# saandeepa93/distributed_compute_pytorch

Measured on AMD Instinct MI355X. Metric: samples/sec (whole node) ResNet-50 DDP at 1/2/4/8 MI355X; scaling efficiency, higher is better.
Workload: dtype bf16; 1 GPU; model=resnet50, global_batch=1024, per_gpu_batch=1024, grad_accum=1, parallelism=dp1, impl=ours, fused_kernels=True, optimizer=SGD, comm_dtype=fp32, hip_graph=False, grad_to_none=True, backend=rccl, mfma_1x1_gemm=True, image_size=224, channels_last=True, res_prologue=False

## Files before the change

csrc/fused.cpp:

```cpp
#include "fused.h"

#include <cstring>

#include <c10/hip/HIPGuard.h>
#include <c10/hip/HIPStream.h>

#include <map>
#include <tuple>
#include <mutex>

#include "common.h"
#include "kernels/bn_kernels.h"
#include "kernels/gemm_kernels.h"
#include "kernels/attn_kernels.h"
#include "kernels/kernels.h"
#include "kernels/ln_kernels.h"
#include "kernels/dropout_kernels.h"
#include "kernels/pool_kernels.h"
#include "kernels/metrics_kernels.h"
#include "kernels/gelu_kernels.h"

namespace dcp {
namespace fused {

// ... 1096 lines not shown
  at::Tensor o = at::empty(q.sizes(), q.options().memory_format(at::MemoryFormat::Contiguous));
  at::Tensor lse = at::empty({q.size(0) * heads, q.size(1)}, q.options().dtype(at::kFloat));
  const bool store = p.p_drop > 0.f && keep_bits;
  at::Tensor mask = at::empty({store ? kern::attn_mask_words(p.B, p.H, p.T) : 0}, q.options().dtype(at::kInt));
  if (store) p.mask = reinterpret_cast<uint32_t*>(mask.data_ptr<int32_t>());
  kern::attn_fwd(p, attn_view(q, "q"), attn_view(k, "k"), attn_view(v, "v"), attn_out(o, "o"), lse.data_ptr<float>(),
                 stream_of(q));
  return {o, lse, mask};
}

void flash_attn_bwd(const at::Tensor& dout, const at::Tensor& q, const at::Tensor& k, const at::Tensor& v,
                    const at::Tensor& o, const at::Tensor& lse, const at::Tensor& mask, int64_t heads, bool causal,
                    double p_drop, int64_t seed, at::Tensor& dq, at::Tensor& dk, at::Tensor& dv,
                    const c10::optional<at::Tensor>& key_mask) {
  for (const at::Tensor* t : std::initializer_list<const at::Tensor*>{&k, &v, &o, &dout, &dq, &dk, &dv})
    same_shape(q, *t, "flash_attn_bwd");
  c10::hip::HIPGuard guard(q.device().index());
  kern::AttnParams p = attn_params(q, heads, causal, p_drop, seed);
  p.kmask = attn_kmask(key_mask, q, p, "flash_attn_bwd");
  DK_CHECK(lse.scalar_type() == at::kFloat && lse.is_contiguous() && lse.numel() == q.size(0) * heads * q.size(1),
            "flash_attn_bwd: lse");
  if (p.p_drop > 0.f) {
    DK_CHECK(mask.is_cuda() && mask.scalar_type() == at::kInt && mask.is_contiguous() &&
                 mask.numel() == kern::attn_mask_words(p.B, p.H, p.T),
             "flash_attn_bwd: dropout keep bits of the forward required");
    p.mask = reinterpret_cast<uint32_t*>(const_cast<int32_t*>(mask.data_ptr<int32_t>()));
  }
  at::Tensor delta = at::empty_like(lse);
  kern::attn_bwd(p, attn_view(q, "q"), attn_view(k, "k"), attn_view(v, "v"), attn_view(o, "o"),
                 attn_view(dout, "dout"), lse.data_ptr<float>(), delta.data_ptr<float>(), attn_out(dq, "dq"),
                 attn_out(dk, "dk"), attn_out(dv, "dv"), stream_of(q));
}

namespace {
float* fptr(const c10::optional<at::Tensor>& t) {
  return (t.has_value() && t->defined()) ? t->data_ptr<float>() : nullptr;
}
}

std::vector<at::Tensor> bn_resbn_act_fwd(const at::Tensor& x, const at::Tensor& weight, const at::Tensor& bias,
                                         const c10::optional<at::Tensor>& running_mean,
                                         const c10::optional<at::Tensor>& running_var,
                                         const c10::optional<at::Tensor>& nbt, const at::Tensor& stats,
                                         const at::Tensor& x2, const at::Tensor& weight2, const at::Tensor& bias2,
                                         const c10::optional<at::Tensor>& running_mean2,
                                         const c10::optional<at::Tensor>& running_var2,
                                         const c10::optional<at::Tensor>& nbt2, const at::Tensor& stats2,
                                         double momentum, double eps, double momentum2, double eps2) {
  check_nhwc(x, "bn_resbn_act_fwd");
  check_nhwc(x2, "bn_resbn_act_fwd(x2)");
  c10::hip::HIPGuard guard(x.device().index());
  const int64_t C = x.size(1);
  const int64_t M = x.numel() / C;
  DK_CHECK(x2.sizes() == x.sizes() && x2.scalar_type() == x.scalar_type(), "bn_resbn_act_fwd: x2 mismatch");
  for (const at::Tensor* t : {&stats, &stats2})
    DK_CHECK(t->scalar_type() == at::kFloat && t->numel() == 2 * C && t->is_contiguous(),
              "bn_resbn_act_fwd: stats must be fp32 [2*C]");
  for (const at::Tensor* t : {&weight, &bias, &weight2, &bias2})
    DK_CHECK(t->scalar_type() == at::kFloat && t->numel() == C && t->is_contiguous(),
              "bn_resbn_act_fwd: affine parameters must be fp32 [C]");
  auto fopt = x.options().dtype(at::kFloat);
  at::Tensor y = at::empty_like(x, cl_fmt(x));
  at::Tensor mean = at::empty({C}, fopt), invstd = at::empty({C}, fopt);
  at::Tensor mean2 = at::empty({C}, fopt), invstd2 = at::empty({C}, fopt);
  at::Tensor bits = at::empty({M * C / 8}, x.options().dtype(at::kByte));
  kern::ResBnArgs rb;
  rb.acc = stats2.data_ptr<float>();
  rb.gamma = weight2.data_ptr<float>();
  rb.beta = bias2.data_ptr<float>();
  rb.mean_out = mean2.data_ptr<float>();
  rb.invstd_out = invstd2.data_ptr<float>();
  rb.running_mean = fptr(running_mean2);
  rb.running_var = fptr(running_var2);
  rb.momentum = static_cast<float>(momentum2);
  rb.eps = static_cast<float>(eps2);
  rb.nbt = nbt2.has_value() && nbt2->defined() ? nbt2->data_ptr<int64_t>() : nullptr;
  kern::bn_forward_train_resbn(bn_dtype(x), x.data_ptr(), x2.data_ptr(), y.data_ptr(), M, static_cast<int>(C),
                               weight.data_ptr<float>(), bias.data_ptr<float>(), fptr(running_mean),
                               fptr(running_var), static_cast<float>(momentum), static_cast<float>(eps),
                               mean.data_ptr<float>(), invstd.data_ptr<float>(), stats.data_ptr<float>(),
                               nbt.has_value() && nbt->defined() ? nbt->data_ptr<int64_t>() : nullptr,
                               bits.data_ptr<uint8_t>(), rb, stream_of(x));
  return {y, mean, invstd, bits, mean2, invstd2};
}

std::vector<at::Tensor> bn_resbn_act_bwd(const at::Tensor& gy, const c10::optional<at::Tensor>& gy2_opt,
                                         const at::Tensor& x, const at::Tensor& weight, const at::Tensor& mean,
                                         const at::Tensor& invstd, const at::Tensor& bits, const at::Tensor& x2,
                                         const at::Tensor& weight2, const at::Tensor& mean2,
                                         const at::Tensor& invstd2) {
  check_nhwc(x, "bn_resbn_act_bwd");
  c10::hip::HIPGuard guard(x.device().index());
  at::Tensor g = gy.contiguous(cl_fmt(x));
  if (g.scalar_type() != x.scalar_type()) g = g.to(x.scalar_type());
  at::Tensor g2;
  if (gy2_opt.has_value() && gy2_opt->defined()) {
    g2 = gy2_opt->contiguous(cl_fmt(x));
    if (g2.scalar_type() != x.scalar_type()) g2 = g2.to(x.scalar_type());
  }
  const int64_t C = x.size(1);
  const int64_t M = x.numel() / C;
  DK_CHECK(bits.numel() == M * C / 8, "bn_resbn_act_bwd: relu bits mismatch");
  auto fopt = x.options().dtype(at::kFloat);
  auto s = stream_of(x);
  at::Tensor gout = at::empty_like(x, cl_fmt(x));
  at::Tensor dx = at::empty_like(x, cl_fmt(x)), dx2 = at::empty_like(x2, cl_fmt(x2));
  at::Tensor dw = at::empty({C}, fopt), db = at::empty({C}, fopt), dw2 = at::empty({C}, fopt),
             db2 = at::empty({C}, fopt);
  at::Tensor acc = zeroed_floats(2 * C, x, s), acc2 = zeroed_floats(2 * C, x, s);
  kern::bn_backward_resbn(bn_dtype(x), g.data_ptr(), g2.defined() ? g2.data_ptr() : nullptr, x.data_ptr(), M,
                          static_cast<int>(C), weight.data_ptr<float>(), mean.data_ptr<float>(),
                          invstd.data_ptr<float>(), bits.data_ptr<uint8_t>(), gout.data_ptr(), dx.data_ptr(),
                          dw.data_ptr<float>(), db.data_ptr<float>(), acc.data_ptr<float>(), x2.data_ptr(),
                          mean2.data_ptr<float>(), acc2.data_ptr<float>(), s);
  kern::bn_backward_apply_plain(bn_dtype(x), gout.data_ptr(), x2.data_ptr(), M, static_cast<int>(C),
                                weight2.data_ptr<float>(), mean2.data_ptr<float>(), invstd2.data_ptr<float>(),
                                acc2.data_ptr<float>(), dx2.data_ptr(), dw2.data_ptr<float>(),
                                db2.data_ptr<float>(), s);
  return {dx, dw, db, dx2, dw2, db2};
}

std::vector<at::Tensor> bn_act_bwd(const at::Tensor& gy, const c10::optional<at::Tensor>& gy2_opt,
                                   const at::Tensor& x, const c10::optional<at::Tensor>& weight,
                                   const c10::optional<at::Tensor>& bias, const at::Tensor& mean,
                                   const at::Tensor& invstd, const at::Tensor& y, bool act, bool has_res,
                                   bool training, const c10::optional<at::Tensor>& relu_bits) {
  check_nhwc(x, "bn_act_bwd");
  c10::hip::HIPGuard guard(x.device().index());
  at::Tensor g = gy.contiguous(cl_fmt(x));
  if (g.scalar_type() != x.scalar_type()) g = g.to(x.scalar_type());
  at::Tensor g2;
  if (gy2_opt.has_value() && gy2_opt->defined()) {
    g2 = gy2_opt->contiguous(cl_fmt(x));
    if (g2.scalar_type() != x.scalar_type()) g2 = g2.to(x.scalar_type());
    if (!has_res) {
      g = g + g2;
      g2 = at::Tensor();
    }
  }
  const int64_t C = x.size(1);
  const int64_t M = x.numel() / C;
  auto fopt = x.options().dtype(at::kFloat);
  at::Tensor dx = at::empty_like(x, cl_fmt(x));
  at::Tensor gres = has_res ? at::empty_like(x, cl_fmt(x)) : at::Tensor();
  const bool has_w = weight.has_value() && weight->defined();
  at::Tensor w = has_w ? weight->to(at::kFloat).contiguous() : at::Tensor();
  const bool has_bias = bias.has_value() && bias->defined();
  at::Tensor bf = has_bias ? bias->to(at::kFloat).contiguous() : at::Tensor();
  at::Tensor dw = at::empty({C}, fopt);
  at::Tensor db = at::empty({C}, fopt);
  at::Tensor acc = zeroed_floats(2 * C, x, stream_of(x));
  kern::bn_backward(bn_dtype(x), g.data_ptr(), g2.defined() ? g2.data_ptr() : nullptr, y.data_ptr(), x.data_ptr(),
                    M, static_cast<int>(C),
                    has_w ? w.data_ptr<float>() : nullptr, bf.defined() ? bf.data_ptr<float>() : nullptr,
                    mean.data_ptr<float>(), invstd.data_ptr<float>(), act,
                    has_res, has_res ? gres.data_ptr() : nullptr, dx.data_ptr(), dw.data_ptr<float>(),
                    db.data_ptr<float>(), acc.data_ptr<float>(), training,
                    relu_bits.has_value() && relu_bits->defined() && relu_bits->numel() == M * C / 8
                        ? relu_bits->data_ptr<uint8_t>()
                        : nullptr,
                    stream_of(x));
  at::Tensor dweight = has_w ? dw.to(weight->scalar_type()) : at::Tensor();
  const bool has_b = bias.has_value() && bias->defined();
  at::Tensor dbias = has_b ? db.to(bias->scalar_type()) : at::Tensor();
  return {dx, dweight, dbias, gres};
}
// ... 391 lines not shown
  m.def("bn_supported", [](int64_t C) { return kern::bn_supported(static_cast<int>(C)); });
  m.def("layer_norm_supported", &layer_norm_supported);
  m.def("linear_dgrad_gelu", &linear_dgrad_gelu, pybind11::arg("gy"), pybind11::arg("w2t"), pybind11::arg("h"),
        pybind11::arg("tanh_approx"), pybind11::arg("accumulate_into") = pybind11::none(),
        pybind11::arg("pp") = false);
  m.def("layer_norm_fwd", &layer_norm_fwd, pybind11::arg("x"), pybind11::arg("weight"), pybind11::arg("bias"),
        pybind11::arg("eps"), pybind11::arg("out_dtype") = pybind11::none(), pybind11::arg("branch") = pybind11::none(),
        pybind11::arg("p") = 0.0, pybind11::arg("seed") = 0, pybind11::arg("offset_dev") = pybind11::none());
  m.def("layer_norm_bwd", &layer_norm_bwd, pybind11::arg("dy"), pybind11::arg("x"), pybind11::arg("weight"),
        pybind11::arg("bias"), pybind11::arg("mean"), pybind11::arg("rstd"),
        pybind11::arg("accumulate_into") = pybind11::none(), pybind11::arg("grad_residual") = pybind11::none(),
        pybind11::arg("dy2") = pybind11::none(), pybind11::arg("drop_p") = 0.0, pybind11::arg("drop_seed") = 0,
        pybind11::arg("drop_offset_dev") = pybind11::none(), pybind11::arg("branch_grad") = false);
  m.def("cross_entropy_fwd", &cross_entropy_fwd, pybind11::arg("logits"), pybind11::arg("target"),
        pybind11::arg("ignore_index"), pybind11::arg("label_smoothing"), pybind11::arg("n_valid") = -1);
  m.def("log_softmax_fwd", &log_softmax_fwd, pybind11::arg("x"), pybind11::arg("out_dtype") = pybind11::none());
  m.def("log_softmax_bwd", &log_softmax_bwd);
  m.def("cross_entropy_bwd", &cross_entropy_bwd, pybind11::arg("logits"), pybind11::arg("target"),
        pybind11::arg("lse"), pybind11::arg("dloss"), pybind11::arg("ignore_index"), pybind11::arg("label_smoothing"),
        pybind11::arg("n_valid") = -1, pybind11::arg("inplace") = false);
  m.def("bn_act_fwd", &bn_act_fwd, "fused NHWC BatchNorm(+residual)(+ReLU) forward", pybind11::arg("x"),
        pybind11::arg("weight"), pybind11::arg("bias"), pybind11::arg("running_mean"), pybind11::arg("running_var"),
        pybind11::arg("residual"), pybind11::arg("training"), pybind11::arg("momentum"), pybind11::arg("eps"),
        pybind11::arg("act"), pybind11::arg("num_batches_tracked") = pybind11::none(),
        pybind11::arg("stats") = pybind11::none());
  m.def("bn_stats_coef", &bn_stats_coef, "training BN statistics + folded scale/shift (no apply)",
        pybind11::arg("x"), pybind11::arg("weight"), pybind11::arg("bias"), pybind11::arg("running_mean"),
        pybind11::arg("running_var"), pybind11::arg("momentum"), pybind11::arg("eps"),
        pybind11::arg("num_batches_tracked") = pybind11::none(), pybind11::arg("sums") = pybind11::none());
  m.def("conv1x1_supported", &conv1x1_supported);
  m.def("conv1x1_fwd", &conv1x1_fwd, "NHWC 1x1 conv as an MFMA GEMM (+BN-apply prologue, +BN-stats epilogue)",
        pybind11::arg("x"), pybind11::arg("w"), pybind11::arg("scale") = pybind11::none(),
        pybind11::arg("shift") = pybind11::none(), pybind11::arg("relu") = false, pybind11::arg("stats") = false);
  m.def("conv1x1_dgrad", &conv1x1_dgrad, pybind11::arg("gy"), pybind11::arg("wt"));
  m.def("conv1x1_fwd_res", &conv1x1_fwd_res, "block boundary: conv1x1(relu(x*scale+shift+res), w) with y and its "
        "ReLU mask stored by the GEMM's prologue", py::arg("x"), py::arg("w"), py::arg("scale"), py::arg("shift"),
        py::arg("res"), py::arg("stats") = true);
  m.def("lm_head_xent_fwd", &lm_head_xent_fwd,
        "LM head GEMM with the cross-entropy's softmax partials in its epilogue -> (logits, loss, lse)",
        py::arg("x"), py::arg("w"), py::arg("target"), py::arg("ignore_index"), py::arg("V"));
  m.def("gemm_pp", &gemm_pp, "x·wᵀ (+bias) (+gelu) on the 8-wave ping-pong 256x256 MFMA GEMM", py::arg("x"),
        py::arg("w"), py::arg("bias") = py::none(), py::arg("gelu") = 0);
  m.def("linear_fwd", &linear_fwd, "Linear forward on the MFMA GEMM: bias (+ GELU tanh/erf) in the epilogue",
        pybind11::arg("x"), pybind11::arg("w"), pybind11::arg("b"), pybind11::arg("gelu") = 0);
  m.def("attn_ok", &attn_ok);
  m.def("embedding_small_bwd", &embedding_small_bwd, "gw += per-index row sums (embedding tables of <= 8 rows)",
        pybind11::arg("idx"), pybind11::arg("g"), pybind11::arg("gw"));
  m.def("colsum", &colsum, "fp32 column sums of a bf16 [.., N] tensor (bias gradient)", pybind11::arg("x"),
        pybind11::arg("accumulate_into") = pybind11::none());
  m.def("colsum_multi", &colsum_multi, "colsum over 1-4 bf16 row segments in one launch", pybind11::arg("xs"),
        pybind11::arg("accumulate_into") = pybind11::none());
  m.def("gelu_fwd", &gelu_fwd, "bf16 GELU forward (erf or tanh form)", pybind11::arg("h"),
        pybind11::arg("tanh_approx"));
  m.def("gelu_bwd", &gelu_bwd, "bf16 GELU backward (+ fused bias-gradient column sums)", pybind11::arg("gy"),
        pybind11::arg("h"), pybind11::arg("tanh_approx"), pybind11::arg("bias_grad"),
        pybind11::arg("accumulate_into") = pybind11::none());
  m.def("flash_attn_fwd", &flash_attn_fwd, "MFMA flash attention forward (head dim 64)", pybind11::arg("q"),
        pybind11::arg("k"), pybind11::arg("v"), pybind11::arg("heads"), pybind11::arg("causal"),
        pybind11::arg("p_drop"), pybind11::arg("seed"), pybind11::arg("keep_bits") = true,
        pybind11::arg("key_mask") = pybind11::none());
  m.def("flash_attn_bwd", &flash_attn_bwd, "MFMA flash attention backward into dq/dk/dv", pybind11::arg("dout"),
        pybind11::arg("q"), pybind11::arg("k"), pybind11::arg("v"), pybind11::arg("o"), pybind11::arg("lse"),
        pybind11::arg("keep"), pybind11::arg("heads"), pybind11::arg("causal"), pybind11::arg("p_drop"),
        pybind11::arg("seed"), pybind11::arg("dq"), pybind11::arg("dk"), pybind11::arg("dv"),
        pybind11::arg("key_mask") = pybind11::none());
  m.def("attn_pack_key_mask", &attn_pack_key_mask,
        "bool [B, T] key-padding mask -> packed int64 [B, 1 + T/64] for flash_attn_fwd / flash_attn_bwd",
        pybind11::arg("mask"));
  m.def("conv_fwd", &conv_fwd, "kxk NHWC conv forward (implicit-GEMM MFMA) [+ output BN sums]", pybind11::arg("x"),
        pybind11::arg("wt"), pybind11::arg("kh"), pybind11::arg("kw"), pybind11::arg("stride"), pybind11::arg("pad"),
        pybind11::arg("stats") = false);
  m.def("conv1x1_dgrad_bnred", &conv1x1_dgrad_bnred, "1x1 data gradient + BN/ReLU backward reduction epilogue");
  m.def("conv_dgrad_bnred", &conv_dgrad_bnred, "stride-1 kxk data gradient + BN/ReLU backward reduction epilogue");
  m.def("conv1x1_dgrad_resred", &conv1x1_dgrad_resred,
        "1x1 data gradient + residual BN(+RBN)/ReLU backward reduction epilogue -> (g, acc, acc2)",
        pybind11::arg("gy"), pybind11::arg("wt"), pybind11::arg("x"), pybind11::arg("gy2"), pybind11::arg("mean"),
        pybind11::arg("bits"), pybind11::arg("x2") = pybind11::none(), pybind11::arg("mean2") = pybind11::none());
  m.def("bn_bwd_apply_g", &bn_bwd_apply_g, "BN training backward apply from a masked gradient + its reduction");
  m.def("conv3_bwd_fused", &conv3_bwd_fused,
        "bottleneck conv3 backward with BN3's backward apply as its prologue -> (dy2, acc2, dz3)");
  m.def("conv3_bwd_mode", [](int64_t M, int64_t w) { return kern::conv3_bwd_mode(M, static_cast<int>(w)); },
        "0: conv3's backward of this shape stays unfused; 1: conv3_bwd_fused");
  m.def("bn_dparams", &bn_dparams, "(dweight, dbias) of a training BN from its backward reduction");
  m.def("bn_bwd_apply2_g", &bn_bwd_apply2_g,
        "both BNs of relu(bn(x) + bn2(x2)) backward from the shared masked gradient in one pass");
  m.def("bn_act_bwd_apply", &bn_act_bwd_apply, "BN/ReLU training backward apply from a precomputed reduction");
  m.def("bn_resbn_act_fwd", &bn_resbn_act_fwd, "training relu(bn(x) + bn2(x2)), both BNs fused (downsample block)");
  m.def("bn_resbn_act_bwd", &bn_resbn_act_bwd, "backward of bn_resbn_act_fwd");
  m.def("conv1x1_s2_dgrad", &conv1x1_s2_dgrad, "stride-2 1x1 conv data gradient (GEMM + scattering epilogue)");
  m.def("conv_dgrad_s2_multi", &conv_dgrad_s2_multi,
        "3x3 stride-2 pad-1 conv data gradient: four parity classes in one implicit-GEMM launch");
  m.def("conv_dgrad_s2", &conv_dgrad_s2, "stride-2 kxk conv data gradient as four parity-class implicit GEMMs");
  m.def("conv_wgrad", &conv_wgrad, "kxk NHWC conv weight gradient (implicit-GEMM MFMA, fp32 out)",
        pybind11::arg("gy"), pybind11::arg("x"), pybind11::arg("kh"), pybind11::arg("kw"), pybind11::arg("stride"),
        pybind11::arg("pad"));
  m.def("weight_bf16_t", &weight_bf16_t, "fp32 weight -> (bf16 [R,C], bf16 transposed [C,R]) in one launch");
  m.def("conv_weight_bf16", &conv_weight_bf16, "kxk weight -> (bf16 fwd [Co][kh][kw][Ci], bf16 flipped [Ci][kh][kw][Co])");
  m.def("weight_prep_plan", &weight_prep_plan,
        "conv / Linear weights -> (device table, tiles, bf16 fwd views, bf16 dgrad views), one view pair per group "
        "(a group of Linear weights is packed along its rows)",
        py::arg("weights"), py::arg("groups") = std::vector<int64_t>{}, py::arg("pad_rows") = std::vector<int64_t>{});
  m.def("weight_prep_run", &weight_prep_run, py::arg("table"), py::arg("tiles"));
  m.def("conv1x1_wgrad", &conv1x1_wgrad, pybind11::arg("gy"), pybind11::arg("x"),
        pybind11::arg("scale") = pybind11::none(), pybind11::arg("shift") = pybind11::none(),
        pybind11::arg("relu") = false, pybind11::arg("accumulate_into") = pybind11::none(),
        pybind11::arg("out_rows") = -1, pybind11::arg("slots") = 0);
  m.def("conv1x1_wgrad_multi", &conv1x1_wgrad_multi,
        "dW = sum over 1-4 (gy, x) row segments (gradient-accumulation micro-steps) in one wgrad launch",
        pybind11::arg("gys"), pybind11::arg("xs"), pybind11::arg("accumulate_into") = pybind11::none(),
        pybind11::arg("out_rows") = -1);
  m.def("bn_act_bwd", &bn_act_bwd, "fused NHWC BatchNorm(+residual)(+ReLU) backward", pybind11::arg("gy"),
        pybind11::arg("gy2"), pybind11::arg("x"), pybind11::arg("weight"), pybind11::arg("bias"),
        pybind11::arg("mean"), pybind11::arg("invstd"), pybind11::arg("y"), pybind11::arg("act"),
        pybind11::arg("has_res"), pybind11::arg("training"), pybind11::arg("relu_bits") = pybind11::none());
}

}
}
```

csrc/kernels/gemm.hip:

```cpp
#include <hip/hip_runtime.h>

#include <cstdlib>
#include <string>

#include "gelu_math.h"
#include "gemm_kernels.h"
#include "kernels.h"
#include "stem_kernels.h"

namespace dcp {
namespace kern {
namespace {

typedef __bf16 bf16x8 __attribute__((ext_vector_type(8)));
typedef short s16x4 __attribute__((ext_vector_type(4)));
typedef short s16x8 __attribute__((ext_vector_type(8)));
typedef float f32x4 __attribute__((ext_vector_type(4)));
typedef __attribute__((address_space(3))) s16x4 lds_s16x4;

constexpr int kT = 256;
int g_wg_slots = 512;
int g_wg_cap = 0;
constexpr int kBK = 32;
constexpr int kNS = 4;
// ... 1518 lines not shown
        const int row = wi * 32 + i * 16 + (lane >> 4) * 4 + r;
        const int col = (j >> 1) * C + wj * 32 + (j & 1) * 16 + (lane & 15);
        out[static_cast<int64_t>(row) * COLS + col] = acc[i][j][r];
      }
}

struct WgradPlan {
  int bm, bn, tiles, S;
  int64_t chunk;
};

inline int wgrad_order() { return 1; }

inline bool wgrad_mtap(int N2, int taps) { return taps > 1 && N2 == 64; }

WgradPlan wgrad_plan(int64_t M, int N1, int N2, int taps = 1) {
  WgradPlan p;
  p.bm = N1 % 128 == 0 ? 128 : 64;
  p.bn = N2 % 128 == 0 ? 128 : 64;
  p.tiles = (N1 / p.bm) * (N2 / p.bn);
  constexpr int kStep = 64;
  const int64_t ksteps = (M + kStep - 1) / kStep;
  const int64_t slots = (g_wg_cap == 0 && taps > 1 && M <= 65536) ? 2 * g_wg_slots : g_wg_slots;
  int64_t S = slots / (p.tiles * taps);
  const int64_t capx = g_wg_cap > 0 ? g_wg_cap : (M <= 65536 ? 4 : 1);
  const int64_t cap = capx * (M * (N1 + static_cast<int64_t>(taps) * N2) * 2 / 2) /
                      (static_cast<int64_t>(N1) * taps * N2 * 4);
  if (S > cap) S = cap;
  if (S > ksteps) S = ksteps;
  if (S < 1) S = 1;
  p.chunk = ((ksteps + S - 1) / S) * kStep;
  p.S = static_cast<int>((M + p.chunk - 1) / p.chunk);
  return p;
}

}

bool gemm_nt_supported(int64_t M, int64_t N, int64_t K) {
  return M >= 1 && N > 0 && K > 0 && N % 64 == 0 && K % 64 == 0 && K <= 4096;
}

namespace {
inline int nt_bk() { return 64; }

inline int nt_bm(int64_t M, int tn, int BN, bool pro, int K, bool gather) {
  if (BN == 64) return !gather && K >= 256 ? 256 : 128;
  return pro && (M / 256) * tn >= 256 ? 256 : 128;
}

}

namespace {
int g_nt_big = 2;
int g_lin_big = 1;
int g_big_pipe = 0;
int g_nt_a = 0;
int g_stem_wide = 1;
int g_slab32 = 1;
int g_nt_deep = 0;
int g_pro_pipe = 0;
int g_reserve_cus = [] {
  const char* v = getenv("DCP_RESERVE_CUS");
  const int r = v ? atoi(v) : 0;
  return r < 0 ? 0 : (r > 192 ? 192 : r);
}();
inline int grid_cus() { return 256 - g_reserve_cus; }
}
void gemm_tune(const char* key, int value) {
  const std::string k(key);
  if (k == "nt_big") g_nt_big = value;
  if (k == "lin_big") g_lin_big = value;
  if (k == "big_pipe") g_big_pipe = value;
  if (k == "nt_a") g_nt_a = value < 0 ? 0 : (value > 3 ? 3 : value);
  if (k == "stem_wide") g_stem_wide = value;
  if (k == "slab32") g_slab32 = value;
  if (k == "nt_deep") g_nt_deep = value;
  if (k == "pro_pipe") g_pro_pipe = value;
  if (k == "wg_slots") g_wg_slots = value < 64 ? 64 : value;
  if (k == "wg_cap") g_wg_cap = value < 0 ? 0 : value;
  if (k == "reserve_cus") g_reserve_cus = value < 0 ? 0 : (value > 192 ? 192 : value);
  if (k.rfind("pp_", 0) == 0) gemm_pp_tune(key, value);
  if (k.rfind("bn_", 0) == 0) bn_tune(key, value);
  if (k.rfind("c3bwd", 0) == 0) conv3_bwd_tune(key, value);
  wgrad_pp_tune(key, value);
}
int gemm_tune_get(const char* key) {
  const std::string k(key);
  if (k == "nt_big") return g_nt_big;
  if (k == "lin_big") return g_lin_big;
  if (k == "big_pipe") return g_big_pipe;
  if (k == "nt_a") return g_nt_a;
  if (k == "stem_wide") return g_stem_wide;
  if (k == "slab32") return g_slab32;
  if (k == "nt_deep") return g_nt_deep;
  if (k == "pro_pipe") return g_pro_pipe;
  if (k == "wg_slots") return g_wg_slots;
  if (k == "wg_cap") return g_wg_cap;
  if (k == "reserve_cus") return g_reserve_cus;
  if (k.rfind("pp_", 0) == 0) return gemm_pp_tune_get(key);
  if (k.rfind("bn_", 0) == 0) return bn_tune_get(key);
  if (k.rfind("c3bwd", 0) == 0) return conv3_bwd_tune_get(key);
  return wgrad_pp_tune_get(key);
}

namespace {
template <bool GATHER, int BK, int BM>
void gemm_nt_launch_bm(const void* A, const void* B, void* C, int64_t M, int N, int K, const float* scale,
                       const float* shift, bool relu, float* stats, const ConvGeo& geo, const BnRedArgs* red,
                       hipStream_t s, bool scatter2, bool parity) {
  const int BN = N % 128 == 0 ? 128 : 64;
  const int tiles_m = static_cast<int>((M + BM - 1) / BM);
  const int tn = N / BN;
  const int kRes = (BM == 128 ? 2 : 1) * grid_cus();
  const int64_t tiles = static_cast<int64_t>(tiles_m) * tn;
  int P = tiles <= kRes ? static_cast<int>(tiles) : (kRes / tn) * tn;
  if (P < tn) P = tn;
  const dim3 grid(P);
  const bool pro = scale != nullptr;
  const bool st = stats != nullptr;
  const int nw = (BM / 64) * (BN == 64 && BM == 256 ? 1 : 2);
  const size_t lds = static_cast<size_t>(nt_stages<BK>()) * (BM + BN) * BK * 2 +
                     static_cast<size_t>(nw) * 32 * (BN * 2 / (BM == 256 && BN == 64 ? 1 : 2)) +
                     (pro ? 8 * static_cast<size_t>(K) : 0);
  const int NT = 64 * nw;
  auto a = static_cast<const uint16_t*>(A);
  auto b = static_cast<const uint16_t*>(B);
  auto c = static_cast<uint16_t*>(C);
  const BnRedArgs bnr = red ? *red : BnRedArgs{};
#define DK_GNT(BN_, P_, S_)                                                                                     \
  hipLaunchKernelGGL((gemm_nt_kernel<BM, BN_, P_, S_, GATHER, BK>), grid, dim3(NT), lds, s, a, b, c, M, N, K,   \
                     scale, shift, relu ? 1 : 0, stats, tiles_m, tn, geo, bnr)
#define DK_GNT2(BN_)                            \
  do {                                           \
    if (red) {                                   \
      if constexpr (!GATHER) {                   \
        if (red->bits && red->x2) {              \
          DK_GNT(BN_, false, 6);                \
          break;                                 \
        }                                        \
        if (red->bits) {                         \
          DK_GNT(BN_, false, 5);                \
          break;                                 \
        }                                        \
      }                                          \
      DK_GNT(BN_, false, 2);                    \
      break;                                     \
    }                                            \
    if constexpr (!GATHER) {                     \
      if (scatter2) {                            \
        DK_GNT(BN_, false, 3);                  \
        break;                                   \
      }                                          \
    } else {                                     \
      if (parity) {                              \
        DK_GNT(BN_, false, 4);                  \
        break;                                   \
      }                                          \
    }                                            \
    if constexpr (!GATHER) {                     \
      if (pro && st) {                           \
        DK_GNT(BN_, true, 1);                   \
        break;                                   \
      }                                          \
      if (pro) {                                 \
        DK_GNT(BN_, true, 0);                   \
        break;                                   \
      }                                          \
    }                                            \
    if (st) DK_GNT(BN_, false, 1);              \
    else DK_GNT(BN_, false, 0);                 \
  } while (0)
  if (BN == 128) DK_GNT2(128);
  else DK_GNT2(64);
#undef DK_GNT2
#undef DK_GNT
}

template <int BM>
void gemm_nt_res_launch(const void* A, const void* B, void* C, int64_t M, int N, int K, const float* scale,
                        const float* shift, float* stats, const BnRedArgs& bnr, hipStream_t s) {
  constexpr int BK = 32;
  const int BN = N % 128 == 0 ? 128 : 64;
  const int tiles_m = static_cast<int>((M + BM - 1) / BM);
  const int tn = N / BN;
// ... 771 lines not shown
```

csrc/kernels/kernels.h:

```cpp
#pragma once

#include <hip/hip_runtime.h>

#include <cstdint>

namespace dcp {
namespace kern {

enum DType : int { F32 = 0, BF16 = 1, F16 = 2 };

constexpr int64_t kChunk = 8192;

struct TableView {
  const int64_t* base;
  int n;
};

void mt_copy(TableView t, int64_t nchunks, DType src, DType dst, float scale, hipStream_t s);

void mt_sgd(TableView t, int64_t nchunks, DType p, float lr, float momentum, float dampening, float wd,
            bool nesterov, bool maximize, bool first_step, bool has_buf, float grad_scale, hipStream_t s);

void mt_adam(TableView t, int64_t nchunks, DType p, float lr, float beta1, float beta2, float eps, float wd,
             float bias_c1, float bias_c2_sqrt, bool amsgrad, bool decoupled_wd, bool maximize, float grad_scale,
             bool shadow, int step_list, hipStream_t s);

void mt_adadelta(TableView t, int64_t nchunks, DType p, float lr, float rho, float eps, float wd, bool maximize,
                 float grad_scale, hipStream_t s);

void mt_sumsq(TableView t, int64_t nchunks, DType d, float* out, hipStream_t s);
bool emb_small_supported(int64_t V, int64_t D);
void emb_small_bwd(const int64_t* idx, const float* g, float* gw, int64_t M, int V, int D, hipStream_t s);

void mt_scale_by(TableView t, int64_t nchunks, DType d, const float* scale_dev, hipStream_t s);

void copy_words(const int64_t* src, int64_t* dst, int64_t n, hipStream_t s);

void comm_emulate(const void* src, void* scratch, int64_t bytes_buf, int64_t bytes_move, int channels, double us,
                  hipStream_t s);

void conv3_bwd_bf16(const void* g, const void* z3, const void* wt, const void* x2, void* dz3, void* dy2, int64_t M,
                    int w, const float* gamma3, const float* mean3, const float* invstd3, const float* acc3,
                    const float* gamma2, const float* beta2, const float* mean2, const float* invstd2, float* stats,
                    hipStream_t s);
int conv3_bwd_mode(int64_t M, int w);
bool conv3_bwd_tune(const char* key, int value);
int conv3_bwd_tune_get(const char* key);
void bn_dparams(const float* acc, const float* invstd, float* dgamma, float* dbeta, int C, hipStream_t s);

}
}
```

csrc/selftest/kern_stubs.cpp:

```cpp
#include <cstdio>
#include <cstdlib>

#include "kernels/kernels.h"

namespace dcp {
namespace kern {
namespace {
[[noreturn]] void gpu_only(const char* f) {
  std::fprintf(stderr, "%s: GPU launcher reached from a CPU self-test\n", f);
  std::abort();
}
}

void mt_copy(TableView, int64_t, DType, DType, float, hipStream_t) { gpu_only("mt_copy"); }
void mt_sgd(TableView, int64_t, DType, float, float, float, float, bool, bool, bool, bool, float, hipStream_t) {
  gpu_only("mt_sgd");
}
void mt_adam(TableView, int64_t, DType, float, float, float, float, float, float, float, bool, bool, bool, float, bool,
             int, hipStream_t) {
  gpu_only("mt_adam");
}
void mt_adadelta(TableView, int64_t, DType, float, float, float, float, bool, float, hipStream_t) {
  gpu_only("mt_adadelta");
}
void mt_sumsq(TableView, int64_t, DType, float*, hipStream_t) { gpu_only("mt_sumsq"); }
void mt_scale_by(TableView, int64_t, DType, const float*, hipStream_t) { gpu_only("mt_scale_by"); }
void copy_words(const int64_t*, int64_t*, int64_t, hipStream_t) { gpu_only("copy_words"); }
void conv3_bwd_bf16(const void*, const void*, const void*, const void*, void*, void*, int64_t, int, const float*,
                    const float*, const float*, const float*, const float*, const float*, const float*, const float*,
                    float*, hipStream_t) {
  gpu_only("conv3_bwd_bf16");
}
int conv3_bwd_mode(int64_t, int) { return 0; }
bool conv3_bwd_tune(const char*, int) { return false; }
int conv3_bwd_tune_get(const char*) { return -1; }
void bn_dparams(const float*, const float*, float*, float*, int, hipStream_t) { gpu_only("bn_dparams"); }

}
}
```

distributed_compute_pytorch_amd/ops/conv.py:

```python
from __future__ import annotations

from typing import Optional, Tuple

import torch
import torch.nn.functional as F

from .._ext import C as _C


def _cl(t: torch.Tensor) -> torch.Tensor:
    if t.dtype != torch.bfloat16:
        t = t.to(torch.bfloat16)
    return t.contiguous(memory_format=torch.channels_last) if t.dim() == 4 else t.contiguous()


_PREPPED = {}


class ConvWeightPrep:

    def __init__(self, weights):
        self.weights = list(weights)
        self._key = None

# ... 82 lines not shown
                           "gradient it received is not that boundary's deferred one (z3 has another consumer?); "
                           "gemm_tune c3bwd=0 disables the fusion")
    return e[1:]


def _c3_defer_ok(z3: torch.Tensor) -> bool:
    fn = z3.grad_fn
    if fn is None or not torch.is_grad_enabled() or z3.dtype != torch.bfloat16 or z3.dim() != 4:
        return False
    if isinstance(fn, _BNReluConv1x1Fn._backward_cls):
        if not _PRO_RED:
            return False
    elif isinstance(fn, _BNReluConvFn._backward_cls):
        if fn.cfg[0] != 1 or fn.cfg[1] != 1:
            return False
    else:
        return False
    c = z3.shape[1]
    if c % 4 or not z3.is_contiguous(memory_format=torch.channels_last):
        return False
    if _C.conv3_bwd_mode(z3.numel() // c, c // 4) <= 0:
        return False
    fn._c3_defer = True
    return True


_PRO_RED = True


class _BNReluConv1x1Fn(torch.autograd.Function):
    @staticmethod
    def forward(ctx, x, gamma, beta, weight, running_mean, running_var, nbt, momentum, eps, stats, sums):
        mean, invstd, scale, shift = _C.bn_stats_coef(x, gamma, beta, running_mean, running_var, float(momentum),
                                                      float(eps), nbt, sums)
        w, wt = _w2d(weight)
        z, st = _C.conv1x1_fwd(x, w, scale, shift, True, bool(stats))
        ctx.save_for_backward(x, gamma, beta, wt, mean, invstd, scale, shift)
        ctx.wshape, ctx.wdtype = weight.shape, weight.dtype
        ctx.mark_non_differentiable(st)
        ctx.set_materialize_grads(False)
        return z, st

    @staticmethod
    def backward(ctx, gz, _gst):
        x, gamma, beta, wt, mean, invstd, scale, shift = ctx.saved_tensors
        if gz is None:
            return (None,) * 11
        gz = _cl(gz)
        d3 = _c3_take(ctx, gz)
        if d3 is not None:
            da, acc, gz = _C.conv3_bwd_fused(gz, *d3, wt, x, gamma, beta, mean, invstd)
        dw = _C.conv1x1_wgrad(gz, x, scale, shift, True).view(ctx.wshape)
        if dw.dtype != ctx.wdtype:
            dw = dw.to(ctx.wdtype)
        if d3 is not None:
            dx, dgamma, dbeta = _C.bn_act_bwd_apply(da, x, gamma, beta, mean, invstd, acc)
        elif _PRO_RED:
            da, acc = _C.conv1x1_dgrad_bnred(gz, wt, x, gamma, beta, mean, invstd)
            dx, dgamma, dbeta = _C.bn_act_bwd_apply(da, x, gamma, beta, mean, invstd, acc)
        else:
            da = _C.conv1x1_dgrad(gz, wt)
            dx, dgamma, dbeta, _ = _C.bn_act_bwd(da, None, x, gamma, beta, mean, invstd, x, True, False, True, None)
        return dx, dgamma, dbeta, dw, None, None, None, None, None, None, None


def conv1x1(x: torch.Tensor, weight: torch.Tensor, stats: bool = False) -> Tuple[torch.Tensor, Optional[torch.Tensor]]:
    return _Conv1x1Fn.apply(x, weight, stats)


def bn_relu_conv1x1(x: torch.Tensor, bn, weight: torch.Tensor, stats: bool = False,
                    sums: Optional[torch.Tensor] = None):
    nbt = bn.num_batches_tracked
    if nbt is not None and (nbt.device != x.device or nbt.dtype != torch.int64):
        nbt.add_(1)
        nbt = None
    return _BNReluConv1x1Fn.apply(x, bn.weight, bn.bias, weight, bn.running_mean, bn.running_var, nbt, bn.momentum,
                                  bn.eps, stats, sums)


_APPLY2 = True
RES_PROLOGUE = False


class _BNResActConv1x1Fn(torch.autograd.Function):

    @staticmethod
    def forward(ctx, z3, gamma, beta, residual, x2, gamma2, beta2, w_next, rm, rv, nbt, stats, rm2, rv2, nbt2,
                stats2, momentum, eps, momentum2, eps2, defer=False):
        ctx.set_materialize_grads(False)
        ctx.defer = bool(defer) and x2 is None
        if x2 is not None:
            y, mean, invstd, bits, mean2, invstd2 = _C.bn_resbn_act_fwd(
                z3, gamma, beta, rm, rv, nbt, stats, x2, gamma2, beta2, rm2, rv2, nbt2, stats2, float(momentum),
                float(eps), float(momentum2), float(eps2))
            w, wt = _w2d(w_next)
            z1, s1 = _C.conv1x1_fwd(y, w, None, None, False, True)
        elif RES_PROLOGUE:
            mean, invstd, scale, shift = _C.bn_stats_coef(z3, gamma, beta, rm, rv, float(momentum), float(eps), nbt,
                                                          stats)
            w, wt = _w2d(w_next)
            z1, s1, y, bits = _C.conv1x1_fwd_res(z3, w, scale, shift, _cl(residual), True)
            mean2 = invstd2 = None
        else:
            y, mean, invstd, bits = _C.bn_act_fwd(z3, gamma, beta, rm, rv, residual, True, float(momentum),
                                                  float(eps), True, nbt, stats)
            mean2 = invstd2 = None
            w, wt = _w2d(w_next)
            z1, s1 = _C.conv1x1_fwd(y, w, None, None, False, True)
        ctx.save_for_backward(z3, gamma, mean, invstd, bits, y, wt, x2, gamma2, mean2, invstd2)
        ctx.wshape, ctx.wdtype = w_next.shape, w_next.dtype
        ctx.mark_non_differentiable(s1)
        return y, z1, s1

    @staticmethod
    def backward(ctx, gy, gz, _gs):
        z3, gamma, mean, invstd, bits, y, wt, x2, gamma2, mean2, invstd2 = ctx.saved_tensors
        if gz is None:
            gz = torch.zeros((y.shape[0], ctx.wshape[0]) + tuple(y.shape[2:]), device=y.device, dtype=y.dtype)
        gz = _cl(gz)
        dw = _C.conv1x1_wgrad(gz, y)
        g, acc, acc2 = _C.conv1x1_dgrad_resred(gz, wt, z3, None if gy is None else _cl(gy), mean, bits, x2, mean2)
        dres = dx2 = dgamma2 = dbeta2 = None
        if x2 is not None and _APPLY2:
            dz3, dgamma, dbeta, dx2, dgamma2, dbeta2 = _C.bn_bwd_apply2_g(g, z3, gamma, mean, invstd, acc, x2, gamma2,
                                                                          mean2, invstd2, acc2)
        elif ctx.defer:
            _c3_put(g, z3, gamma, mean, invstd, acc)
            dz3 = dres = g
            dgamma, dbeta = _C.bn_dparams(acc, invstd)
        else:
            dz3, dgamma, dbeta = _C.bn_bwd_apply_g(g, z3, gamma, mean, invstd, acc)
            if x2 is not None:
                dx2, dgamma2, dbeta2 = _C.bn_bwd_apply_g(g, x2, gamma2, mean2, invstd2, acc2)
            else:
                dres = g
        dw = dw.view(ctx.wshape)
        if dw.dtype != ctx.wdtype:
            dw = dw.to(ctx.wdtype)
        return (dz3, dgamma, dbeta, dres, dx2, dgamma2, dbeta2, dw) + (None,) * 13


def bn_res_act_conv1x1(bn3, z3: torch.Tensor, s3: torch.Tensor, identity: Optional[torch.Tensor], w_next,
                       resbn=None):

    def _nbt(m):
        t = m.num_batches_tracked
        if t is not None and (t.device != z3.device or t.dtype != torch.int64):
            t.add_(1)
            return None
        return t

    if resbn is not None:
        bn_d, x2, s2 = resbn
        return _BNResActConv1x1Fn.apply(z3, bn3.weight, bn3.bias, None, x2, bn_d.weight, bn_d.bias, w_next,
                                        bn3.running_mean, bn3.running_var, _nbt(bn3), s3, bn_d.running_mean,
                                        bn_d.running_var, _nbt(bn_d), s2, bn3.momentum, bn3.eps, bn_d.momentum,
                                        bn_d.eps)
    return _BNResActConv1x1Fn.apply(z3, bn3.weight, bn3.bias, identity, None, None, None, w_next, bn3.running_mean,
                                    bn3.running_var, _nbt(bn3), s3, None, None, None, None, bn3.momentum, bn3.eps,
                                    0.0, 0.0, not RES_PROLOGUE and _c3_defer_ok(z3))


def res_conv_fuse_ok(bn3, z3: torch.Tensor, s3, next_conv) -> bool:
    return (bn3.training and bn3.affine and bn3.track_running_stats and bn3.momentum is not None
            and s3 is not None and s3.numel() == 2 * z3.shape[1] and bn3.weight.dtype == torch.float32
            and next_conv.kernel_size == (1, 1) and next_conv.stride == (1, 1) and next_conv.bias is None
            and next_conv.groups == 1 and next_conv.in_channels == z3.shape[1]
            and next_conv.out_channels % 64 == 0 and next_conv.weight.dtype == torch.float32
            and gemm_ok(z3, next_conv.in_channels, next_conv.out_channels))


class _BNReluConvFn(torch.autograd.Function):

    @staticmethod
# ... 175 lines not shown
```

Baseline: 15190 samples/s.

## Fuse block-boundary BN+residual+ReLU with next conv1 forward in one kernel

Adds a kernel that applies BN3 (and optionally the downsample BN), the residual add and ReLU to each tile, writes y and the ReLU mask, and feeds the same tile from LDS into an MFMA 1x1 GEMM producing the next conv1 output and its BN sums. This replaces a separate bn_act/bn_resbn pass followed by a conv1x1_fwd, so y is not re-read from memory for the GEMM and one launch is saved. It applies to K/N shapes 256x64, 512x128 and 256x128, is on by default, and uses a persistent grid with the whole weight held in registers, which may limit occupancy. Stats atomics are now done per workgroup.

```diff
diff --git a/csrc/fused.cpp b/csrc/fused.cpp
--- a/csrc/fused.cpp
+++ b/csrc/fused.cpp
@@ -1202,6 +1202,72 @@
                                nbt.has_value() && nbt->defined() ? nbt->data_ptr<int64_t>() : nullptr,
                                bits.data_ptr<uint8_t>(), rb, stream_of(x));
   return {y, mean, invstd, bits, mean2, invstd2};
+}
+
+std::vector<at::Tensor> conv1_fwd_fused(const at::Tensor& z3, const at::Tensor& w, const at::Tensor& weight,
+                                        const at::Tensor& bias, const c10::optional<at::Tensor>& running_mean,
+                                        const c10::optional<at::Tensor>& running_var,
+                                        const c10::optional<at::Tensor>& nbt, const at::Tensor& stats, double momentum,
+                                        double eps, const c10::optional<at::Tensor>& residual,
+                                        const c10::optional<at::Tensor>& x2, const c10::optional<at::Tensor>& weight2,
+                                        const c10::optional<at::Tensor>& bias2,
+                                        const c10::optional<at::Tensor>& running_mean2,
+                                        const c10::optional<at::Tensor>& running_var2,
+                                        const c10::optional<at::Tensor>& nbt2,
+                                        const c10::optional<at::Tensor>& stats2, double momentum2, double eps2) {
+  check_gemm_act(z3, "conv1_fwd_fused");
+  c10::hip::HIPGuard guard(z3.device().index());
+  DK_CHECK(z3.dim() == 4, "conv1_fwd_fused: z3 must be a channels_last 4-D tensor");
+  const int64_t K = z3.size(1);
+  const int64_t M = z3.numel() / K;
+  DK_CHECK(w.scalar_type() == at::kBFloat16 && w.is_contiguous() && w.numel() % K == 0 && w.device() == z3.device(),
+            "conv1_fwd_fused: weight must be contiguous bf16 [N][K]");
+  const int64_t N = w.numel() / K;
+  DK_CHECK(kern::conv1_fwd_mode(M, static_cast<int>(K), static_cast<int>(N)) > 0, "conv1_fwd_fused: unsupported shape");
+  const bool rbn = x2.has_value() && x2->defined();
+  const bool ident = residual.has_value() && residual->defined();
+  DK_CHECK(rbn != ident, "conv1_fwd_fused: exactly one of residual and x2 is required");
+  const at::Tensor& res = rbn ? *x2 : *residual;
+  check_gemm_act(res, "conv1_fwd_fused");
+  DK_CHECK(res.sizes() == z3.sizes() && res.device() == z3.device(), "conv1_fwd_fused: residual / x2 must match z3");
+  auto f32c = [&](const at::Tensor& t, int64_t n) {
+    return t.scalar_type() == at::kFloat && t.numel() == n && t.is_contiguous() && t.device() == z3.device();
+  };
+  DK_CHECK(f32c(weight, K) && f32c(bias, K) && f32c(stats, 2 * K),
+            "conv1_fwd_fused: BN3 weight / bias fp32 [K], stats fp32 [2*K]");
+  auto nbt_ptr = [](const c10::optional<at::Tensor>& t) {
+    return t.has_value() && t->defined() ? t->data_ptr<int64_t>() : nullptr;
+  };
+  auto fopt = z3.options().dtype(at::kFloat);
+  auto s = stream_of(z3);
+  at::Tensor c3 = at::empty({4, K}, fopt);
+  kern::bn_stats_coef(kern::BN_BF16, z3.data_ptr(), M, static_cast<int>(K), weight.data_ptr<float>(),
+                      bias.data_ptr<float>(), fptr(running_mean), fptr(running_var), static_cast<float>(momentum),
+                      static_cast<float>(eps), c3[0].data_ptr<float>(), c3[1].data_ptr<float>(),
+                      c3[2].data_ptr<float>(), c3[3].data_ptr<float>(), stats.data_ptr<float>(), nbt_ptr(nbt), s, true);
+  at::Tensor cd;
+  if (rbn) {
+    DK_CHECK(weight2.has_value() && bias2.has_value() && stats2.has_value() && f32c(*weight2, K) &&
+                  f32c(*bias2, K) && f32c(*stats2, 2 * K),
+              "conv1_fwd_fused: downsample BN weight / bias fp32 [K], stats fp32 [2*K]");
+    cd = at::empty({4, K}, fopt);
+    kern::bn_stats_coef(kern::BN_BF16, res.data_ptr(), M, static_cast<int>(K), weight2->data_ptr<float>(),
+                        bias2->data_ptr<float>(), fptr(running_mean2), fptr(running_var2),
+                        static_cast<float>(momentum2), static_cast<float>(eps2), cd[0].data_ptr<float>(),
+                        cd[1].data_ptr<float>(), cd[2].data_ptr<float>(), cd[3].data_ptr<float>(),
+                        stats2->data_ptr<float>(), nbt_ptr(nbt2), s, true);
+  }
+  at::Tensor y = at::empty_like(z3, at::MemoryFormat::ChannelsLast);
+  at::Tensor bits = at::empty({M * K / 8}, z3.options().dtype(at::kByte));
+  at::Tensor z1 = at::empty({z3.size(0), N, z3.size(2), z3.size(3)},
+                            z3.options().memory_format(at::MemoryFormat::ChannelsLast));
+  at::Tensor s1 = zeroed_floats(2 * N, z3, s);
+  kern::conv1_fwd_bf16(z3.data_ptr(), res.data_ptr(), w.data_ptr(), y.data_ptr(), bits.data_ptr<uint8_t>(),
+                       z1.data_ptr(), M, static_cast<int>(K), static_cast<int>(N), c3[2].data_ptr<float>(),
+                       c3[3].data_ptr<float>(), rbn ? cd[2].data_ptr<float>() : nullptr,
+                       rbn ? cd[3].data_ptr<float>() : nullptr, s1.data_ptr<float>(), s);
+  if (rbn) return {y, bits, z1, s1, c3[0], c3[1], cd[0], cd[1]};
+  return {y, bits, z1, s1, c3[0], c3[1]};
 }
 
 std::vector<at::Tensor> bn_resbn_act_bwd(const at::Tensor& gy, const c10::optional<at::Tensor>& gy2_opt,
@@ -1759,6 +1825,20 @@
   m.def("conv3_bwd_mode", [](int64_t M, int64_t w) { return kern::conv3_bwd_mode(M, static_cast<int>(w)); },
         "0: conv3's backward of this shape stays unfused; 1: conv3_bwd_fused");
   m.def("bn_dparams", &bn_dparams, "(dweight, dbias) of a training BN from its backward reduction");
+  m.def("conv1_fwd_fused", &conv1_fwd_fused,
+        "block boundary relu(bn3(z3) + residual-or-bn_d(x2)) with the next conv1 fed from the same tile -> "
+        "(y, bits, z1, sums1, mean, invstd[, mean2, invstd2])",
+        pybind11::arg("z3"), pybind11::arg("w"), pybind11::arg("weight"), pybind11::arg("bias"),
+        pybind11::arg("running_mean"), pybind11::arg("running_var"), pybind11::arg("num_batches_tracked"),
+        pybind11::arg("stats"), pybind11::arg("momentum"), pybind11::arg("eps"),
+        pybind11::arg("residual") = pybind11::none(), pybind11::arg("x2") = pybind11::none(),
+        pybind11::arg("weight2") = pybind11::none(), pybind11::arg("bias2") = pybind11::none(),
+        pybind11::arg("running_mean2") = pybind11::none(), pybind11::arg("running_var2") = pybind11::none(),
+        pybind11::arg("num_batches_tracked2") = pybind11::none(), pybind11::arg("stats2") = pybind11::none(),
+        pybind11::arg("momentum2") = 0.0, pybind11::arg("eps2") = 0.0);
+  m.def("conv1_fwd_mode",
+        [](int64_t M, int64_t K, int64_t N) { return kern::conv1_fwd_mode(M, static_cast<int>(K), static_cast<int>(N)); },
+        "0: the block boundary + conv1 forward of this shape stays unfused; 1: conv1_fwd_fused");
   m.def("bn_bwd_apply2_g", &bn_bwd_apply2_g,
         "both BNs of relu(bn(x) + bn2(x2)) backward from the shared masked gradient in one pass");
   m.def("bn_act_bwd_apply", &bn_act_bwd_apply, "BN/ReLU training backward apply from a precomputed reduction");
diff --git a/csrc/kernels/conv1_fwd.hip b/csrc/kernels/conv1_fwd.hip
--- /dev/null
+++ b/csrc/kernels/conv1_fwd.hip
@@ -0,0 +1,257 @@
+#include <hip/hip_runtime.h>
+
+#include <cstring>
+
+#include "kernels.h"
+
+namespace dcp {
+namespace kern {
+namespace {
+
+typedef __bf16 bf16x8 __attribute__((ext_vector_type(8)));
+typedef __bf16 bf16x2 __attribute__((ext_vector_type(2)));
+typedef float f32x4 __attribute__((ext_vector_type(4)));
+typedef unsigned int u32x4 __attribute__((ext_vector_type(4)));
+
+constexpr int kBM = 32;
+
+int g_mode64 = 1;
+int g_mode128 = 1;
+int g_mode256x128 = 1;
+int g_grid = 0;
+
+__device__ __forceinline__ float bf_lo(uint32_t w) { return __uint_as_float(w << 16); }
+__device__ __forceinline__ float bf_hi(uint32_t w) { return __uint_as_float(w & 0xffff0000u); }
+__device__ __forceinline__ uint32_t pack2(float a, float b) {
+  const bf16x2 v = {static_cast<__bf16>(a), static_cast<__bf16>(b)};
+  return __builtin_bit_cast(uint32_t, v);
+}
+__device__ __forceinline__ uint4 ld16_nt(const uint16_t* p) {
+  const u32x4 v = __builtin_nontemporal_load(reinterpret_cast<const u32x4*>(p));
+  return make_uint4(v.x, v.y, v.z, v.w);
+}
+__device__ __forceinline__ void st16_nt(uint16_t* p, uint4 v) {
+  const u32x4 w = {v.x, v.y, v.z, v.w};
+  __builtin_nontemporal_store(w, reinterpret_cast<u32x4*>(p));
+}
+
+struct C1Args {
+  const uint16_t* z3;
+  const uint16_t* res;
+  const uint16_t* w;
+  uint16_t* y;
+  uint8_t* bits;
+  uint16_t* z1;
+  const float* sc;
+  const float* sf;
+  const float* rsc;
+  const float* rsf;
+  float* stats;
+  int64_t M;
+  int tiles;
+};
+
+template <int K, int N, bool RBN>
+__global__ void __launch_bounds__(4 * N) conv1_fwd_kernel(const C1Args a) {
+  constexpr int T = 4 * N;
+  constexpr int CPR = K / 8;
+  constexpr int RPP = T / CPR;
+  constexpr int NP = kBM / RPP;
+  constexpr int KS = K / 32;
+  constexpr int FM = kBM / 16;
+  static_assert(RPP * NP == kBM && CPR % 16 == 0 && T % CPR == 0, "tile shape");
+  __shared__ __attribute__((aligned(16))) char sA[kBM * K * 2];
+
+  const int t = threadIdx.x, lane = t & 63, wv = t >> 6;
+  const int cc = t % CPR, r0 = t / CPR;
+  const int64_t M = a.M;
+
+  const int P = gridDim.x, wid = blockIdx.x;
+  const int xcd = wid & 7, q8 = P >> 3, r8 = P & 7;
+  const int wg = (xcd < r8 ? xcd * (q8 + 1) : r8 * (q8 + 1) + (xcd - r8) * q8) + (wid >> 3);
+
+  float sc[8], sf[8], rsc[RBN ? 8 : 1], rsf[RBN ? 8 : 1];
+#pragma unroll
+  for (int k = 0; k < 8; ++k) {
+    const int c = cc * 8 + k;
+    sc[k] = a.sc[c];
+    sf[k] = a.sf[c];
+    if (RBN) {
+      rsc[k] = a.rsc[c];
+      rsf[k] = a.rsf[c];
+    }
+  }
+  bf16x8 wf[KS];
+  {
+    const uint16_t* wp = a.w + static_cast<int64_t>(16 * wv + (lane & 15)) * K + 8 * (lane >> 4);
+#pragma unroll
+    for (int ks = 0; ks < KS; ++ks) wf[ks] = *reinterpret_cast<const bf16x8*>(wp + 32 * ks);
+  }
+  const int nc = 16 * wv + 4 * (lane >> 4);
+  float ssum[4], ssq[4];
+#pragma unroll
+  for (int r = 0; r < 4; ++r) ssum[r] = ssq[r] = 0.f;
+
+  uint4 zq[NP], rq[NP];
+  auto load = [&](int tl) {
+    const int64_t m0 = static_cast<int64_t>(tl) * kBM;
+#pragma unroll
+    for (int i = 0; i < NP; ++i) {
+      const int64_t m = m0 + r0 + RPP * i;
+      const int64_t o = (m < M ? m : 0) * K + cc * 8;
+      zq[i] = ld16_nt(a.z3 + o);
+      rq[i] = ld16_nt(a.res + o);
+    }
+  };
+
+  int tl = wg;
+  if (tl < a.tiles) load(tl);
+  for (; tl < a.tiles; tl += P) {
+    const int64_t m0 = static_cast<int64_t>(tl) * kBM;
+#pragma unroll
+    for (int i = 0; i < NP; ++i) {
+      const int row = r0 + RPP * i;
+      const int64_t m = m0 + row;
+      const uint32_t z4[4] = {zq[i].x, zq[i].y, zq[i].z, zq[i].w};
+      const uint32_t r4[4] = {rq[i].x, rq[i].y, rq[i].z, rq[i].w};
+      float d[8];
+      uint32_t bits = 0;
+#pragma unroll
+      for (int k = 0; k < 8; ++k) {
+        const float zk = (k & 1) ? bf_hi(z4[k >> 1]) : bf_lo(z4[k >> 1]);
+        const float rk = (k & 1) ? bf_hi(r4[k >> 1]) : bf_lo(r4[k >> 1]);
+        float o = fmaf(zk, sc[k], sf[k]);
+        o += RBN ? fmaf(rk, rsc[RBN ? k : 0], rsf[RBN ? k : 0]) : rk;
+        bits |= (o > 0.f ? 1u : 0u) << k;
+        d[k] = fmaxf(o, 0.f);
+      }
+      uint4 v = make_uint4(pack2(d[0], d[1]), pack2(d[2], d[3]), pack2(d[4], d[5]), pack2(d[6], d[7]));
+      if (m < M) {
+        st16_nt(a.y + m * K + cc * 8, v);
+        a.bits[m * CPR + cc] = static_cast<uint8_t>(bits);
+      } else {
+        v = make_uint4(0, 0, 0, 0);
+      }
+      *reinterpret_cast<uint4*>(sA + row * (K * 2) + 16 * (cc ^ (row & 15))) = v;
+    }
+    __syncthreads();
+    if (tl + P < a.tiles) load(tl + P);
+
+    f32x4 acc[FM];
+#pragma unroll
+    for (int j = 0; j < FM; ++j) acc[j] = f32x4{0.f, 0.f, 0.f, 0.f};
+#pragma unroll
+    for (int ks = 0; ks < KS; ++ks) {
+#pragma unroll
+      for (int j = 0; j < FM; ++j) {
+        const int row = 16 * j + (lane & 15);
+        const bf16x8 xf =
+            *reinterpret_cast<const bf16x8*>(sA + row * (K * 2) + 16 * ((4 * ks + (lane >> 4)) ^ (row & 15)));
+        acc[j] = __builtin_amdgcn_mfma_f32_16x16x32_bf16(wf[ks], xf, acc[j], 0, 0, 0);
+      }
+    }
+#pragma unroll
+    for (int j = 0; j < FM; ++j) {
+      const int64_t m = m0 + 16 * j + (lane & 15);
+      if (m < M) {
+        const uint2 v = make_uint2(pack2(acc[j][0], acc[j][1]), pack2(acc[j][2], acc[j][3]));
+        *reinterpret_cast<uint2*>(a.z1 + m * N + nc) = v;
+        const uint32_t w2[2] = {v.x, v.y};
+#pragma unroll
+        for (int r = 0; r < 4; ++r) {
+          const float zk = (r & 1) ? bf_hi(w2[r >> 1]) : bf_lo(w2[r >> 1]);
+          ssum[r] += zk;
+          ssq[r] = fmaf(zk, zk, ssq[r]);
+        }
+      }
+    }
+    __syncthreads();
+  }
+#pragma unroll
+  for (int r = 0; r < 4; ++r)
+#pragma unroll
+    for (int o = 1; o < 16; o <<= 1) {
+      ssum[r] += __shfl_xor(ssum[r], o);
+      ssq[r] += __shfl_xor(ssq[r], o);
+    }
+  if ((lane & 15) == 0 && wg < a.tiles) {
+#pragma unroll
+    for (int r = 0; r < 4; ++r) {
+      atomicAdd(a.stats + nc + r, ssum[r]);
+      atomicAdd(a.stats + N + nc + r, ssq[r]);
+    }
+  }
+}
+
+int* mode_of(int K, int N) {
+  if (K == 256 && N == 64) return &g_mode64;
+  if (K == 512 && N == 128) return &g_mode128;
+  if (K == 256 && N == 128) return &g_mode256x128;
+  return nullptr;
+}
+
+template <int K, int N>
+void launch(const C1Args& a, bool rbn, int per_cu, hipStream_t s) {
+  int P = 256 * per_cu;
+  if (g_grid > 0 && g_grid < P) P = g_grid;
+  if (P > a.tiles) P = a.tiles;
+  if (rbn) hipLaunchKernelGGL((conv1_fwd_kernel<K, N, true>), dim3(P), dim3(4 * N), 0, s, a);
+  else hipLaunchKernelGGL((conv1_fwd_kernel<K, N, false>), dim3(P), dim3(4 * N), 0, s, a);
+}
+
+}
+
+bool conv1_fwd_tune(const char* key, int value) {
+  const int m = value < 0 ? 0 : (value > 1 ? 1 : value);
+  if (!strcmp(key, "c1fwd")) g_mode64 = g_mode128 = g_mode256x128 = m;
+  else if (!strcmp(key, "c1fwd64")) g_mode64 = m;
+  else if (!strcmp(key, "c1fwd128")) g_mode128 = m;
+  else if (!strcmp(key, "c1fwd256x128")) g_mode256x128 = m;
+  else if (!strcmp(key, "c1fwd_grid")) g_grid = value < 0 ? 0 : value;
+  else return false;
+  return true;
+}
+
+int conv1_fwd_tune_get(const char* key) {
+  if (!strcmp(key, "c1fwd")) {
+    const int m = g_mode64 < g_mode128 ? g_mode64 : g_mode128;
+    return m < g_mode256x128 ? m : g_mode256x128;
+  }
+  if (!strcmp(key, "c1fwd64")) return g_mode64;
+  if (!strcmp(key, "c1fwd128")) return g_mode128;
+  if (!strcmp(key, "c1fwd256x128")) return g_mode256x128;
+  if (!strcmp(key, "c1fwd_grid")) return g_grid;
+  return -1;
+}
+
+int conv1_fwd_mode(int64_t M, int K, int N) {
+  if (M <= 0 || M >= (int64_t(1) << 31)) return 0;
+  const int* m = mode_of(K, N);
+  return m ? *m : 0;
+}
+
+void conv1_fwd_bf16(const void* z3, const void* res, const void* w, void* y, uint8_t* bits, void* z1, int64_t M, int K,
+                    int N, const float* scale, const float* shift, const float* rscale, const float* rshift,
+                    float* stats, hipStream_t s) {
+  C1Args a;
+  a.z3 = static_cast<const uint16_t*>(z3);
+  a.res = static_cast<const uint16_t*>(res);
+  a.w = static_cast<const uint16_t*>(w);
+  a.y = static_cast<uint16_t*>(y);
+  a.bits = bits;
+  a.z1 = static_cast<uint16_t*>(z1);
+  a.sc = scale;
+  a.sf = shift;
+  a.rsc = rscale;
+  a.rsf = rshift;
+  a.stats = stats;
+  a.M = M;
+  a.tiles = static_cast<int>((M + kBM - 1) / kBM);
+  const bool rbn = rscale != nullptr;
+  if (K == 256 && N == 64) launch<256, 64>(a, rbn, 3, s);
+  else if (K == 512 && N == 128) launch<512, 128>(a, rbn, 1, s);
+  else launch<256, 128>(a, rbn, rbn ? 1 : 2, s);
+}
+
+}
+}
diff --git a/csrc/kernels/gemm.hip b/csrc/kernels/gemm.hip
--- a/csrc/kernels/gemm.hip
+++ b/csrc/kernels/gemm.hip
@@ -1624,6 +1624,7 @@
   if (k.rfind("pp_", 0) == 0) gemm_pp_tune(key, value);
   if (k.rfind("bn_", 0) == 0) bn_tune(key, value);
   if (k.rfind("c3bwd", 0) == 0) conv3_bwd_tune(key, value);
+  if (k.rfind("c1fwd", 0) == 0) conv1_fwd_tune(key, value);
   wgrad_pp_tune(key, value);
 }
 int gemm_tune_get(const char* key) {
@@ -1642,6 +1643,7 @@
   if (k.rfind("pp_", 0) == 0) return gemm_pp_tune_get(key);
   if (k.rfind("bn_", 0) == 0) return bn_tune_get(key);
   if (k.rfind("c3bwd", 0) == 0) return conv3_bwd_tune_get(key);
+  if (k.rfind("c1fwd", 0) == 0) return conv1_fwd_tune_get(key);
   return wgrad_pp_tune_get(key);
 }
 
diff --git a/csrc/kernels/kernels.h b/csrc/kernels/kernels.h
--- a/csrc/kernels/kernels.h
+++ b/csrc/kernels/kernels.h
@@ -48,5 +48,12 @@
 int conv3_bwd_tune_get(const char* key);
 void bn_dparams(const float* acc, const float* invstd, float* dgamma, float* dbeta, int C, hipStream_t s);
 
+void conv1_fwd_bf16(const void* z3, const void* res, const void* w, void* y, uint8_t* bits, void* z1, int64_t M, int K,
+                    int N, const float* scale, const float* shift, const float* rscale, const float* rshift,
+                    float* stats, hipStream_t s);
+int conv1_fwd_mode(int64_t M, int K, int N);
+bool conv1_fwd_tune(const char* key, int value);
+int conv1_fwd_tune_get(const char* key);
+
 }
 }
diff --git a/csrc/selftest/kern_stubs.cpp b/csrc/selftest/kern_stubs.cpp
--- a/csrc/selftest/kern_stubs.cpp
+++ b/csrc/selftest/kern_stubs.cpp
@@ -35,6 +35,13 @@
 bool conv3_bwd_tune(const char*, int) { return false; }
 int conv3_bwd_tune_get(const char*) { return -1; }
 void bn_dparams(const float*, const float*, float*, float*, int, hipStream_t) { gpu_only("bn_dparams"); }
+void conv1_fwd_bf16(const void*, const void*, const void*, void*, uint8_t*, void*, int64_t, int, int, const float*,
+                    const float*, const float*, const float*, float*, hipStream_t) {
+  gpu_only("conv1_fwd_bf16");
+}
+int conv1_fwd_mode(int64_t, int, int) { return 0; }
+bool conv1_fwd_tune(const char*, int) { return false; }
+int conv1_fwd_tune_get(const char*) { return -1; }
 
 }
 }
diff --git a/distributed_compute_pytorch_amd/ops/conv.py b/distributed_compute_pytorch_amd/ops/conv.py
--- a/distributed_compute_pytorch_amd/ops/conv.py
+++ b/distributed_compute_pytorch_amd/ops/conv.py
@@ -188,6 +188,28 @@
 RES_PROLOGUE = False
 
 
+def _c1_fused_ok(z3, gamma, beta, stats, res, gamma2, beta2, stats2, w_next) -> bool:
+
+    def act(t):
+        return (t is not None and t.is_cuda and t.dtype == torch.bfloat16 and t.dim() == 4
+                and t.is_contiguous(memory_format=torch.channels_last))
+
+    def vec(t, n):
+        return t is not None and t.dtype == torch.float32 and t.numel() == n and t.is_contiguous()
+
+    if not act(z3) or res is None or res.shape != z3.shape or w_next.dim() != 4 or w_next.shape[2:] != (1, 1):
+        return False
+    k = z3.shape[1]
+    if w_next.shape[1] != k or not (vec(gamma, k) and vec(beta, k) and vec(stats, 2 * k)):
+        return False
+    if gamma2 is not None:
+        if not (act(res) and vec(gamma2, k) and vec(beta2, k) and vec(stats2, 2 * k)):
+            return False
+    elif res.dtype != torch.bfloat16 or res.dim() != 4:
+        return False
+    return _C.conv1_fwd_mode(z3.numel() // k, k, w_next.shape[0]) > 0
+
+
 class _BNResActConv1x1Fn(torch.autograd.Function):
 
     @staticmethod
@@ -195,7 +217,18 @@
                 stats2, momentum, eps, momentum2, eps2, defer=False):
         ctx.set_materialize_grads(False)
         ctx.defer = bool(defer) and x2 is None
-        if x2 is not None:
+        if not RES_PROLOGUE and _c1_fused_ok(z3, gamma, beta, stats, residual if x2 is None else x2, gamma2, beta2,
+                                             stats2, w_next):
+            w, wt = _w2d(w_next)
+            mean2 = invstd2 = None
+            if x2 is not None:
+                y, bits, z1, s1, mean, invstd, mean2, invstd2 = _C.conv1_fwd_fused(
+                    z3, w, gamma, beta, rm, rv, nbt, stats, float(momentum), float(eps), None, x2, gamma2, beta2,
+                    rm2, rv2, nbt2, stats2, float(momentum2), float(eps2))
+            else:
+                y, bits, z1, s1, mean, invstd = _C.conv1_fwd_fused(z3, w, gamma, beta, rm, rv, nbt, stats,
+                                                                   float(momentum), float(eps), _cl(residual))
+        elif x2 is not None:
             y, mean, invstd, bits, mean2, invstd2 = _C.bn_resbn_act_fwd(
                 z3, gamma, beta, rm, rv, nbt, stats, x2, gamma2, beta2, rm2, rv2, nbt2, stats2, float(momentum),
                 float(eps), float(momentum2), float(eps2))
```

Result: faster. 15590 samples/s, median of 6 (+2.7%).
